# songrise/HyperNeRF-torch

Measured on AMD Instinct MI355X. Metric: ray-samples/sec (fwd+bwd+Adam), whole job; per-GPU = value/n_gpus, higher is better.
Workload: dtype bf16

## Files before the change

### hypernerf-torch_amd/csrc/hn_mlp.hip

```cpp
#include "hn_common.h"
#include <algorithm>
#include <type_traits>

#ifdef HN_PROF
#define HN_STAMP(code)                                                                          \
  do {                                                                                          \
    if (prof_on && prof_n < 2040) {                                                             \
      unsigned long long t__;                                                                   \
      __builtin_amdgcn_sched_barrier(0);                                                        \
      asm volatile("s_memtime %0\n\ts_waitcnt lgkmcnt(0)" : "=s"(t__)::"memory");               \
      __builtin_amdgcn_sched_barrier(0);                                                        \
      if (lane == 0) { prof_buf[2 * prof_n] = (code); prof_buf[2 * prof_n + 1] = (long long)t__; } \
      ++prof_n;                                                                                 \
    }                                                                                           \
  } while (0)
#else
#define HN_STAMP(code) do {} while (0)
#endif

template <int WAVES>
struct WStream {
  const char* g;
  char* lds;
  int ctr;
  int nchunks;
  int wave, lane;

  HN_DEV void issue(int c) {
    const char* src = g + (size_t)c * (HN_CHUNK_UNITS * 1024);
    char* dst = lds + (c & 1) * (HN_CHUNK_UNITS * 1024);
    if constexpr (WAVES == 8) {
      if (wave >= 4) {
        int u0 = wave - 4;
        asm volatile("" : "+s"(u0));
#pragma unroll
        for (int i = 0; i < HN_CHUNK_UNITS / 4; ++i) {
          const int unit = u0 + i * 4;
          __builtin_amdgcn_global_load_lds(
              (const __attribute__((address_space(1))) void*)(src + unit * 1024 + lane * 16),
              (__attribute__((address_space(3))) void*)(dst + unit * 1024), 16, 0, 0);
        }
      }
      return;
    }
#pragma unroll
    for (int i = 0; i < HN_CHUNK_UNITS / WAVES; ++i) {
      const int unit = wave + i * WAVES;
      __builtin_amdgcn_global_load_lds(
          (const __attribute__((address_space(1))) void*)(src + unit * 1024 + lane * 16),
          (__attribute__((address_space(3))) void*)(dst + unit * 1024), 16, 0, 0);
    }
  }
  HN_DEV void start() {
    ctr = 0;
    __syncthreads();
    issue(0);
  }
  HN_DEV const char* take(int n) {
    if ((ctr & (HN_CHUNK_UNITS - 1)) + n > HN_CHUNK_UNITS) ctr = (ctr + HN_CHUNK_UNITS - 1) & ~(HN_CHUNK_UNITS - 1);
    if ((ctr & (HN_CHUNK_UNITS - 1)) == 0) {
      const int c = ctr / HN_CHUNK_UNITS;
      asm volatile("s_waitcnt vmcnt(0)" ::: "memory");
      __syncthreads();
      if (c + 1 < nchunks) issue(c + 1);
    }
    const char* p = lds + (((ctr / HN_CHUNK_UNITS) & 1) * HN_CHUNK_UNITS + (ctr & (HN_CHUNK_UNITS - 1))) * 1024;
    ctr += n;
    return p;
  }
};

#define HN_INV2PI_HI 0.15915494309189535f
#define HN_INV2PI_LO ((float)(0.15915494309189535 - (double)0.15915494309189535f))
HN_DEV void hn_rev_split(float x, float& hi, float& lo) {
  hi = __fmul_rn(x, HN_INV2PI_HI);
  lo = __builtin_fmaf(x, HN_INV2PI_LO, __builtin_fmaf(x, HN_INV2PI_HI, -hi));
}
HN_DEV void hn_stage_sources(float* srcv, const HnMlpArgs& a, int p, int ray, int lane, float* rev = nullptr,
                             int n_trig = 0, bool with_lo = true) {
  const int r = lane & 31, h = lane >> 5;
  for (int ci = h; ci < a.n_comps; ci += 2) {
    const int c = a.comps[ci];
    const int sid = c >> 16, col = c & 0xffff;
    HnSrc s = a.src[0];
    if (sid == 1) s = a.src[1];
    if (sid == 2) s = a.src[2];
    if (sid == 3) s = a.src[3];
    float x = 0.0f;
    if (s.ptr != nullptr) {
      long long row = s.per_ray ? ray : p;
      bool ok = true;
      if (s.gather_idx != nullptr) {
        row = s.gather_idx[ray];
        ok = row >= 0 && row < s.gather_rows;
      }
      x = ok ? s.ptr[(size_t)row * s.ld + col] : __builtin_nanf("");
    }
    srcv[ci * 32 + r] = x;
    if (rev != nullptr && ci < n_trig) {
      float hi, lo;
      hn_rev_split(x, hi, lo);
      rev[ci * 32 + r] = hi;
      if (with_lo) rev[(n_trig + ci) * 32 + r] = lo;
    }
  }
  if (rev != nullptr && !with_lo && h == 0) rev[n_trig * 32 + r] = 0.0f;
}

HN_DEV float hn_direct_source(const HnFeat e, const HnMlpArgs& a, int p, int ray) {
  const int sid = (e.packed >> 8) & 15, col = (e.packed >> 24) & 255;
  const float* base = a.src[0].ptr;
  int ld = a.src[0].ld, pr = a.src[0].per_ray;
  if (sid == 1) { base = a.src[1].ptr; ld = a.src[1].ld; pr = a.src[1].per_ray; }
  if (sid == 2) { base = a.src[2].ptr; ld = a.src[2].ld; pr = a.src[2].per_ray; }
  if (sid == 3) { base = a.src[3].ptr; ld = a.src[3].ld; pr = a.src[3].per_ray; }
  return base[(size_t)(pr ? ray : p) * ld + col];
}

HN_DEV float hn_sin_rev(float t) { return __builtin_amdgcn_sinf(__builtin_amdgcn_fractf(t)); }
#define HN_INV_2PI 0.15915494309189535f

struct HnDFeat { unsigned off; float scale, phase; unsigned idmask; };
HN_DEV HnDFeat hn_derive_feat(const HnFeat e) {
  const int kind = (e.packed >> 12) & 15;
  HnDFeat d;
  d.off = (unsigned)(e.packed & 255) * 128u;
  const bool trig = kind == HN_FEAT_SIN || kind == HN_FEAT_COS || kind == HN_FEAT_SINP;
  d.scale = trig ? e.freq * 0.15915494309189535f : 0.0f;
  d.phase = (kind == HN_FEAT_COS || kind == HN_FEAT_SINP) ? 0.25f : 0.0f;
  d.idmask = (kind == HN_FEAT_ID || kind == HN_FEAT_ID_DIRECT) ? 0xffffffffu : 0u;
  return d;
}
HN_DEV HnDFeat hn_derive_feat_fwd(const HnFeat e, int n_comps, int n_trig, bool with_lo) {
  const int kind = (e.packed >> 12) & 15, ci = e.packed & 255;
  HnDFeat d;
  const bool trig = (kind == HN_FEAT_SIN || kind == HN_FEAT_COS || kind == HN_FEAT_SINP) && ci < n_trig;
  const unsigned oa = trig ? (unsigned)(n_comps + ci) * 128u : (unsigned)ci * 128u;
  const unsigned ob = trig ? (unsigned)(n_comps + n_trig + (with_lo ? ci : 0)) * 128u : oa;
  d.off = oa | ob << 16;
  d.scale = trig ? e.freq : 0.0f;
  d.phase = (kind == HN_FEAT_COS || kind == HN_FEAT_SINP) ? 0.25f : 0.0f;
  d.idmask = (kind == HN_FEAT_ID || kind == HN_FEAT_ID_DIRECT) ? 0xffffffffu : 0u;
  return d;
}
HN_DEV float hn_bfi(unsigned m, float a, float b) {
  return __uint_as_float((m & __float_as_uint(a)) | (~m & __float_as_uint(b)));
}
HN_DEV void hn_features4(const HnDFeat* tp, const char* srcv_r, float* out) {
  u32x4 t[4];
#pragma unroll
  for (int j = 0; j < 4; ++j) t[j] = reinterpret_cast<const u32x4*>(tp)[j];
  __builtin_amdgcn_sched_barrier(0);
  float va[4], vb[4];
// ... 33 lines not shown
  const int kind = (e.packed >> 12) & 15;
  if constexpr (DIRECT) {
    if (kind == HN_FEAT_ID_DIRECT) return hn_direct_source(e, a, p, ray);
  }
  const float x = srcv[(e.packed & 255) * 32 + r];
  if constexpr (BF16) {
    const float ph = (kind == HN_FEAT_COS || kind == HN_FEAT_SINP) ? 0.25f : 0.0f;
    const float s = hn_sin_rev(__builtin_fmaf(e.freq * HN_INV_2PI, x, ph));
    return kind == HN_FEAT_ID ? x : (kind == HN_FEAT_ZERO ? 0.0f : s);
  } else {
    if (kind == HN_FEAT_ZERO) return 0.0f;
    if (kind == HN_FEAT_ID) return x;
    float arg = __fmul_rn(e.freq, x);
    if (kind == HN_FEAT_SINP) arg = __fadd_rn(arg, 0.5f * 3.1415926f);
    return kind == HN_FEAT_COS ? cosf(arg) : sinf(arg);
  }
}

template <bool BF16>
HN_DEV float hn_feature_grad(const HnFeat e, const float* srcv, int r) {
  const int kind = (e.packed >> 12) & 15;
  const float x = srcv[(e.packed & 255) * 32 + r];
  if constexpr (BF16) {
    const float ph = (kind == HN_FEAT_COS || kind == HN_FEAT_SINP) ? 0.5f : 0.25f;
    const float g = e.freq * hn_sin_rev(__builtin_fmaf(e.freq * HN_INV_2PI, x, ph));
    return (kind == HN_FEAT_ID || kind == HN_FEAT_ID_DIRECT) ? 1.0f : g;
  } else {
    if (kind == HN_FEAT_ID || kind == HN_FEAT_ID_DIRECT) return 1.0f;
    float arg = __fmul_rn(e.freq, x);
    if (kind == HN_FEAT_SINP) arg = __fadd_rn(arg, 0.5f * 3.1415926f);
    if (kind == HN_FEAT_COS) return -e.freq * sinf(arg);
    return e.freq * cosf(arg);
  }
}

template <bool DIRECT>
HN_DEV void hn_make_group(bf16x8* out, const HnFeat* ft, const HnDFeat* dft, const float* srcv, int lane,
                          const HnMlpArgs& a, int p, int ray) {
  const int h = lane >> 5, r = lane & 31;
  if constexpr (DIRECT) {
#pragma unroll
    for (int s = 0; s < 4; ++s) {
#pragma unroll
      for (int j = 0; j < 8; ++j)
        out[s][j] = (__bf16)hn_feature<true, true>(ft[16 * s + hn_pi16(h, j)], srcv, r, a, p, ray);
    }
  } else {
    const char* srcv_r = reinterpret_cast<const char*>(srcv) + 4 * r;
#pragma unroll
    for (int s = 0; s < 4; ++s) {
      float v[8];
      hn_features4(dft + 16 * s + 4 * h, srcv_r, v);
      hn_features4(dft + 16 * s + 8 + 4 * h, srcv_r, v + 4);
#pragma unroll
      for (int j = 0; j < 8; ++j) out[s][j] = (__bf16)v[j];
    }
  }
}
template <bool DIRECT>
HN_DEV void hn_make_group(float* out, const HnFeat* ft, const HnDFeat*, const float* srcv, int lane, const HnMlpArgs& a,
                          int p, int ray) {
  const int h = lane >> 5, r = lane & 31;
#pragma unroll
  for (int s = 0; s < 32; ++s) {
    out[s] = hn_feature<false, DIRECT>(ft[32 * (s >> 4) + hn_rho(s & 15, h)], srcv, r, a, p, ray);
    if ((s & 7) == 7) __builtin_amdgcn_sched_barrier(0);
  }
}

HN_DEV void hn_init_acc(f32x16& acc, const float* bias, int t, int h) {
  if (bias != nullptr) {
#pragma unroll
    for (int g = 0; g < 4; ++g) {
      const f32x4 b = *reinterpret_cast<const f32x4*>(bias + 32 * t + 8 * g + 4 * h);
      acc[4 * g] = b[0]; acc[4 * g + 1] = b[1]; acc[4 * g + 2] = b[2]; acc[4 * g + 3] = b[3];
    }
  } else {
#pragma unroll
    for (int i = 0; i < 16; ++i) acc[i] = 0.0f;
  }
}

constexpr int HN_PF = 3;
template <bool BF16, int K32>
HN_DEV void hn_gemm_blocks(f32x16& acc, const typename ModeT<BF16>::Frag* in, WStream<ModeT<BF16>::WAVES>& ws) {
  using M = ModeT<BF16>;
  const char* w = ws.take(K32 * M::UNITS32);
  if constexpr (BF16) {
    constexpr int N = 2 * K32;
    constexpr int D = N < HN_PF ? N : HN_PF;
    const char* wl = w + ws.lane * 16;
    bf16x8 q[D];
#pragma unroll
    for (int u = 0; u < D; ++u) q[u] = *reinterpret_cast<const bf16x8*>(wl + u * 1024);
#pragma unroll
    for (int u = 0; u < N; ++u) {
      acc = hn_mfma_bf16(q[u % D], in[u], acc);
      if (u + D < N) q[u % D] = *reinterpret_cast<const bf16x8*>(wl + (u + D) * 1024);
    }
    __builtin_amdgcn_sched_group_barrier(0x100, D, 0);
#pragma unroll
    for (int u = 0; u < N; ++u) {
      __builtin_amdgcn_sched_group_barrier(0x008, 1, 0);
      if (u + D < N) __builtin_amdgcn_sched_group_barrier(0x100, 1, 0);
    }
  } else {
#pragma unroll
    for (int k = 0; k < K32; ++k) hn_mma_block32(acc, w + k * M::UNITS32 * 1024, in + k * M::STEPS32, ws.lane);
  }
}
template <bool BF16>
HN_DEV void hn_gemm_k(f32x16& acc, const typename ModeT<BF16>::Frag* in, int K32, WStream<ModeT<BF16>::WAVES>& ws) {
  if (K32 == 8) hn_gemm_blocks<BF16, 8>(acc, in, ws);
  else if (K32 == 4) hn_gemm_blocks<BF16, 4>(acc, in, ws);
  else if (K32 == 2) hn_gemm_blocks<BF16, 2>(acc, in, ws);
  else if (K32 == 1) hn_gemm_blocks<BF16, 1>(acc, in, ws);
}

template <bool BF16, int S8 = 0>
HN_DEV char* hn_slot_base(const HnMlpArgs& a, int off_kib, int nt, int blk) {
  if (off_kib < 0) return nullptr;
  constexpr int TU = S8 ? 1 : ModeT<BF16>::TILE_UNITS;
  return reinterpret_cast<char*>(a.stash) + (size_t)(unsigned)off_kib * 1024 + (size_t)blk * nt * (TU * 1024);
}
HN_DEV uint32_t* hn_mask_base(const HnMlpArgs& a, int off256, int nt, int blk, int lane) {
  (void)lane;
  return a.masks + (size_t)(unsigned)off256 * 64 + (size_t)blk * nt * 64;
}
HN_DEV int hn_stash_slot(int r, int h, int u) { return 32 * h + (r ^ (4 * h + 8 * u)); }
HN_DEV int hn_stash8_slot(int r, int h) { return (r & 3) + 4 * h + 8 * ((r >> 2) & 1) + 16 * (r >> 3); }
template <int S8>
HN_DEV int hn_cvt2_f8(unsigned w, int old, bool hi) {
  const float lo_f = __uint_as_float(w << 16), hi_f = __uint_as_float(w & 0xffff0000u);
  if constexpr (S8 == 1) return hi ? __builtin_amdgcn_cvt_pk_fp8_f32(lo_f, hi_f, old, true)
                                   : __builtin_amdgcn_cvt_pk_fp8_f32(lo_f, hi_f, old, false);
  else return hi ? __builtin_amdgcn_cvt_pk_bf8_f32(lo_f, hi_f, old, true)
                 : __builtin_amdgcn_cvt_pk_bf8_f32(lo_f, hi_f, old, false);
}
template <int S8>
HN_DEV void hn_stash8_acc(const f32x16& a, char* slot_base, int t, int lane) {
  u32x4 o;
#pragma unroll
  for (int k = 0; k < 4; ++k) {
    int w = 0;
    if constexpr (S8 == 1) {
      w = __builtin_amdgcn_cvt_pk_fp8_f32(a[4 * k], a[4 * k + 1], w, false);
      w = __builtin_amdgcn_cvt_pk_fp8_f32(a[4 * k + 2], a[4 * k + 3], w, true);
    } else {
      w = __builtin_amdgcn_cvt_pk_bf8_f32(a[4 * k], a[4 * k + 1], w, false);
      w = __builtin_amdgcn_cvt_pk_bf8_f32(a[4 * k + 2], a[4 * k + 3], w, true);
    }
    o[k] = (unsigned)w;
  }
  char* dst8 = slot_base + (size_t)t * 1024 + hn_stash8_slot(lane & 31, lane >> 5) * 16;
  __builtin_nontemporal_store(o, reinterpret_cast<u32x4*>(dst8));
}
template <bool BF16, int S8 = 0>
HN_DEV void hn_stash(const typename ModeT<BF16>::Frag* fr, char* slot_base, int t, int lane) {
  using M = ModeT<BF16>;
  if constexpr (BF16 && S8 != 0) {
    const u32x4 f0 = *reinterpret_cast<const u32x4*>(&fr[0]), f1 = *reinterpret_cast<const u32x4*>(&fr[1]);
    u32x4 o;
#pragma unroll
    for (int k = 0; k < 2; ++k) {
      int lo = 0, hi = 0;
      lo = hn_cvt2_f8<S8>(f0[2 * k], lo, false);
      lo = hn_cvt2_f8<S8>(f0[2 * k + 1], lo, true);
      hi = hn_cvt2_f8<S8>(f1[2 * k], hi, false);
      hi = hn_cvt2_f8<S8>(f1[2 * k + 1], hi, true);
      o[k] = (unsigned)lo;
      o[2 + k] = (unsigned)hi;
    }
    char* dst8 = slot_base + (size_t)t * 1024 + hn_stash8_slot(lane & 31, lane >> 5) * 16;
    __builtin_nontemporal_store(o, reinterpret_cast<u32x4*>(dst8));
    return;
  }
  char* dst = slot_base + (size_t)t * (M::TILE_UNITS * 1024);
  if constexpr (BF16) {
    const int off0 = hn_stash_slot(lane & 31, lane >> 5, 0) * 16;
    __builtin_nontemporal_store(*reinterpret_cast<const u32x4*>(&fr[0]), reinterpret_cast<u32x4*>(dst + off0));
    __builtin_nontemporal_store(*reinterpret_cast<const u32x4*>(&fr[1]), reinterpret_cast<u32x4*>(dst + 1024 + (off0 ^ 128)));
  } else {
    const f32x16 z = hn_transpose_tile(fr, lane);
    hn_store_tile(z, dst, lane, (typename M::Frag*)nullptr);
  }
}

template <bool BF16>
HN_DEV unsigned hn_push_mask(unsigned bits, float x) {
  if constexpr (BF16) return __builtin_amdgcn_alignbit(bits, __float_as_uint(x), 31);
  return (bits << 1) | (x > 0.0f ? 0u : 1u);
}
HN_DEV int hn_keep_mask(unsigned nbits, int q, int i) { return (int)(nbits << (16 * q + i)) >> 31; }

template <bool BF16>
// ... 13 lines not shown
    }
  } else if (act == HN_ACT_SOFTPLUS) {
    const float inv = 1.0f / p0;
#pragma unroll 1
    for (int i = 0; i < 16; ++i) {
      const float z = acc[i], u = z * p0;
      const float sp = BF16 ? __logf(1.0f + __expf(u)) : log1pf(expf(u));
      acc[i] = u > p1 ? z : (BF16 ? sp * inv : sp / p0);
    }
  }
}
template <bool BF16>
HN_DEV float hn_dact_y(int act, float y, float p0, float p1) {
  if (act == HN_ACT_ELU) return y > 0.0f ? 1.0f : y + p0;
  const float u = p0 * y;
  return u > p1 ? 1.0f : (BF16 ? 1.0f - __expf(-u) : -expm1f(-u));
}
template <bool BF16>
HN_DEV f32x16 hn_unstash(const char* slot_base, int t, int lane) {
  using M = ModeT<BF16>;
  const char* src = slot_base + (size_t)t * (M::TILE_UNITS * 1024);
  f32x16 y;
  if constexpr (BF16) {
    const int off0 = hn_stash_slot(lane & 31, lane >> 5, 0) * 16;
    const u32x4 f0 = *reinterpret_cast<const u32x4*>(src + off0);
    const u32x4 f1 = *reinterpret_cast<const u32x4*>(src + 1024 + (off0 ^ 128));
#pragma unroll
    for (int k = 0; k < 4; ++k) {
      y[2 * k] = __uint_as_float(f0[k] << 16);
      y[2 * k + 1] = __uint_as_float(f0[k] & 0xffff0000u);
      y[8 + 2 * k] = __uint_as_float(f1[k] << 16);
      y[8 + 2 * k + 1] = __uint_as_float(f1[k] & 0xffff0000u);
    }
  } else {
    float z[16];
#pragma unroll
    for (int g = 0; g < 4; ++g) {
      const f32x4 v = *reinterpret_cast<const f32x4*>(src + g * 1024 + lane * 16);
#pragma unroll
      for (int e = 0; e < 4; ++e) z[4 * g + e] = v[e];
    }
    y = hn_transpose_tile(z, lane);
  }
  return y;
}

typedef const __attribute__((address_space(4))) int* HnOpPtr;
HN_DEV HnOpPtr hn_op_words(const int* ops, int op) {
  return (HnOpPtr)(uintptr_t)(ops + (size_t)op * HN_OP_WORDS);
}
struct HnOpWords {
  int v[HN_OP_WORDS];
  HN_DEV int operator[](int i) const { return v[i]; }
};
HN_DEV HnOpWords hn_load_op(const int* ops, int op, int n_ops) {
  HnOpWords w;
  const HnOpPtr p = hn_op_words(ops, op < n_ops ? op : n_ops - 1);
#pragma unroll
  for (int i = 0; i < HN_OP_WORDS; ++i) w.v[i] = p[i];
  if (op >= n_ops) w.v[0] = -1;
  return w;
}


template <bool TRAIN, int NT, int S8>
HN_DEV void hn_epilogue_share(int k, int tp, f32x16& a, bf16x8* frag, unsigned& bits, char* out_base,
                              uint32_t* mask_base, int lane) {
  if (k < 8) {
#pragma unroll
    for (int e = 0; e < 2; ++e) {
      const int i = 2 * k + e;
      if (TRAIN) bits = hn_push_mask<true>(bits, a[i]);
      frag[i >> 3][i & 7] = (__bf16)__int_as_float(max(__float_as_int(a[i]), 0));
    }
  } else if (TRAIN && k == 8) {
    hn_stash<true, S8>(frag, out_base, tp, lane);
    if ((tp & 1) || tp == NT - 1) {
      mask_base[(tp >> 1) * 64 + lane] = (tp & 1) ? bits : bits << 16;
      bits = 0;
    }
  }
}

template <int K32, int NT, bool TRAIN, int S8>
HN_DEV void hn_layer_pipelined(bf16x8* cur, bf16x8* nxt, const float* bias, WStream<ModeT<true>::WAVES>& ws,
                               char* out_base, uint32_t* mask_base, int lane) {
  constexpr int N = 2 * K32;
  constexpr int D = 2;
  constexpr int SHARES = 9;
  constexpr int PER_SLOT = (SHARES + N - 1) / N;
  const int h = lane >> 5;
  f32x16 acc[2];
  unsigned bits = 0;
#pragma unroll
  for (int t = 0; t <= NT; ++t) {
    const char* wl = nullptr;
    if (t < NT) wl = ws.take(N) + lane * 16;
    const int tp = t - 1;
    bf16x8 q[D];
    if (t < NT) {
      hn_init_acc(acc[t & 1], bias, t, h);
#pragma unroll
      for (int u = 0; u < D; ++u) q[u] = *reinterpret_cast<const bf16x8*>(wl + u * 1024);
    }
    __builtin_amdgcn_sched_barrier(0);
#pragma unroll
    for (int u = 0; u < N; ++u) {
      if (t < NT) {
        acc[t & 1] = hn_mfma_bf16(q[u % D], cur[u], acc[t & 1]);
        if (u + D < N) q[u % D] = *reinterpret_cast<const bf16x8*>(wl + (u + D) * 1024);
      }
      if (t > 0) {
#pragma unroll
        for (int e = 0; e < PER_SLOT; ++e) {
          const int k = u * PER_SLOT + e;
          if (k < SHARES)
            hn_epilogue_share<TRAIN, NT, S8>(k, tp, acc[tp & 1], nxt + tp * 2, bits, out_base, mask_base, lane);
        }
      }
      __builtin_amdgcn_sched_barrier(0);
    }
  }
#pragma unroll
  for (int i = 0; i < NT * 2; ++i) cur[i] = nxt[i];
}

template <bool BF16, int AUXG, bool EXTRA, bool TRAIN, bool S8 = false>
__global__ __launch_bounds__(ModeT<BF16>::WAVES * 64, BF16 ? 2 : 1) void hn_mlp_fwd_kernel(const HnMlpArgs a) {
  using M = ModeT<BF16>;
  constexpr int SX = S8 ? 1 : 0;
  static_assert(!(S8 && (EXTRA || !TRAIN || !BF16)), "the 8-bit stash exists for the render-level bf16 training builds only");
  if constexpr (S8) asm volatile("s_setreg_imm32_b32 hwreg(HW_REG_MODE, 23, 1), 1");
  using Frag = typename M::Frag;
  extern __shared__ __attribute__((aligned(16))) char smem[];
  const int lane = threadIdx.x & 63;
  const int wave = __builtin_amdgcn_readfirstlane(threadIdx.x >> 6);
  const int r = lane & 31, h = lane >> 5;
  constexpr int PTS = M::WAVES * 32;
  const int ntiles = (a.n_points + PTS - 1) / PTS;
  hn_timeline_begin(a.timeline);
#ifdef HN_PROF
  long long* prof_buf = reinterpret_cast<long long*>(a.prof);
  const bool prof_on = prof_buf != nullptr && blockIdx.x == 0 && wave == 0;
  int prof_n = 0;
#endif

  WStream<M::WAVES> ws;
  ws.g = reinterpret_cast<const char*>(a.wstream);
  ws.lds = smem;
  ws.nchunks = a.n_chunks;
  ws.wave = wave;
  ws.lane = lane;

  Frag cur[8 * M::STEPS32];
  Frag nxt[8 * M::STEPS32];

  float* bias_lds = reinterpret_cast<float*>(smem + 2 * HN_CHUNK_UNITS * 1024);
  HnFeat* feat_lds = reinterpret_cast<HnFeat*>(bias_lds + ((a.n_bias + 3) & ~3));
  HnDFeat* dfeat_lds = reinterpret_cast<HnDFeat*>(feat_lds + ((a.n_feat + 1) & ~1));
  const int n_trig = BF16 ? a.n_trig_comps : 0;
  const bool with_lo = a.trig_lo_planes != 0;
  const int n_planes = BF16 ? a.n_comps + n_trig + (with_lo ? n_trig : 1) : a.n_comps;
  float* srcv = reinterpret_cast<float*>(BF16 ? reinterpret_cast<char*>(dfeat_lds + a.n_feat)
                                              : reinterpret_cast<char*>(dfeat_lds)) + wave * (n_planes * 32);
  float* rev = BF16 ? srcv + a.n_comps * 32 : nullptr;
  for (int i = threadIdx.x; i < a.n_bias; i += blockDim.x) bias_lds[i] = a.bias[i];
  for (int i = threadIdx.x; i < a.n_feat; i += blockDim.x) {
    const HnFeat e = a.feat[i];
    feat_lds[i] = e;
    if constexpr (BF16) dfeat_lds[i] = hn_derive_feat_fwd(e, a.n_comps, n_trig, with_lo);
  }
  __syncthreads();

  for (int tile = blockIdx.x; tile < ntiles; tile += gridDim.x) {
    const int blk = tile * M::WAVES + wave;
    const int p0 = blk * 32 + r;
    const bool valid = p0 < a.n_points;
    const int p = valid ? p0 : a.n_points - 1;
    const int ray = p / a.samples_per_ray;
    const bool wave_valid = blk * 32 < a.n_points;
    hn_stage_sources(srcv, a, p, ray, lane, rev, n_trig, with_lo);
    ws.start();

    HnOpWords w_next = hn_load_op(a.ops, 0, a.n_ops);
    for (int op = 0; op < a.n_ops; ++op) {
      const HnOpWords w = w_next;
      w_next = hn_load_op(a.ops, op + 1, a.n_ops);
      const int code = w[0];
      if (code == HN_OP_LAYER) {
        HN_STAMP(100 + op);
        const int K32 = w[1] & 255, nG = (w[1] >> 8) & 255, NT = (w[1] >> 16) & 255;
        const int act = (w[1] >> 24) & 15, flags = (w[1] >> 28) & 15;
        const float* bias = bias_lds + w[2];
        const bool do_mask = TRAIN && w[4] >= 0 && wave_valid && act != HN_ACT_SOFTPLUS;
        const bool do_stash = TRAIN && w[5] >= 0 && wave_valid;
        char* out_base = do_stash ? hn_slot_base<BF16, SX>(a, w[5], NT, blk) : nullptr;
        char* aux_base = (TRAIN && wave_valid) ? hn_slot_base<BF16, SX>(a, w[6], 2 * nG, blk) : nullptr;
        uint32_t* mask_base = do_mask ? hn_mask_base(a, w[4], (NT + 1) >> 1, blk, lane) : nullptr;
        const bool has_out = w_next[0] == HN_OP_OUT;
        const HnOpWords out_w = w_next;
        Frag aux[AUXG * 2 * M::STEPS32];
#pragma unroll
        for (int g = 0; g < AUXG; ++g) {
          if (g < nG) {
            if (EXTRA && (flags & HN_LAYER_DIRECT))
              hn_make_group<true>(aux + g * 2 * M::STEPS32, feat_lds + w[3] + 64 * g, dfeat_lds + w[3] + 64 * g, srcv,
                                  lane, a, p, ray);
            else
              hn_make_group<false>(aux + g * 2 * M::STEPS32, feat_lds + w[3] + 64 * g, dfeat_lds + w[3] + 64 * g, srcv,
                                   lane, a, p, ray);
            if (aux_base != nullptr) {
              hn_stash<BF16, SX>(aux + g * 2 * M::STEPS32, aux_base, 2 * g, lane);
              hn_stash<BF16, SX>(aux + (g * 2 + 1) * M::STEPS32, aux_base, 2 * g + 1, lane);
            }
          }
        }
        unsigned bits = 0;
        HN_STAMP(1);
        if constexpr (BF16) {
          const bool plain = nG == 0 && act == HN_ACT_RELU && !(flags & HN_LAYER_NO_COMMIT) && !has_out &&
                             wave_valid && do_stash == do_mask;
          if (plain && K32 == 4 && NT == 4) {
            if (do_stash) hn_layer_pipelined<4, 4, true, SX>(cur, nxt, bias, ws, out_base, mask_base, lane);
            else hn_layer_pipelined<4, 4, false, SX>(cur, nxt, bias, ws, out_base, mask_base, lane);
            continue;
          }
        }
#pragma unroll
        for (int t = 0; t < 8; ++t) {
          if (t < NT) {
            f32x16 acc;
            hn_init_acc(acc, bias, t, h);
            hn_gemm_k<BF16>(acc, cur, K32, ws);
#pragma unroll
            for (int g = 0; g < AUXG; ++g)
              if (g < nG) hn_gemm_blocks<BF16, 2>(acc, aux + g * 2 * M::STEPS32, ws);
            HN_STAMP(2);
            if (act == HN_ACT_RELU) {
#pragma unroll
              for (int i = 0; i < 16; ++i) {
                bits = hn_push_mask<BF16>(bits, acc[i]);
                acc[i] = __int_as_float(max(__float_as_int(acc[i]), 0));
              }
            } else if (act != HN_ACT_NONE) {
              hn_act_tile<BF16>(acc, act, __int_as_float(w[7]), __int_as_float(w[4]), bits);
            }
            if (has_out && t == 0 && h == 0 && valid) {
              const HnDst d = a.dst[out_w[1]];
              const int n = out_w[3];
#pragma unroll
              for (int i = 0; i < 4; ++i) {
                if (i < n) {
                  float y = acc[i];
                  if (out_w[4] == 1) y = 1.0f / (1.0f + expf(-y));
                  if (out_w[5] >= 0) {
                    const HnSrc sr = a.src[out_w[5]];
                    y = __fadd_rn(sr.ptr[(size_t)(sr.per_ray ? ray : p) * sr.ld + out_w[6] + i], y);
                  }
                  d.ptr[(size_t)p * d.ld + out_w[2] + i] = y;
                }
              }
            }
            if (has_out && t == 0 && h == 0 && out_w[7] > 0) {
              const int n = out_w[3];
#pragma unroll
              for (int i = 0; i < 4; ++i) {
                if (i < n) {
                  float y = acc[i];
                  if (out_w[4] == 1) y = 1.0f / (1.0f + expf(-y));
                  if (out_w[5] >= 0) {
                    const HnSrc sr = a.src[out_w[5]];
                    y = __fadd_rn(sr.ptr[(size_t)(sr.per_ray ? ray : p) * sr.ld + out_w[6] + i], y);
                  }
                  const int ci = out_w[7] - 1 + i;
                  srcv[ci * 32 + r] = y;
                  if (BF16 && ci < n_trig) {
                    float hi, lo;
                    hn_rev_split(y, hi, lo);
                    rev[ci * 32 + r] = hi;
                    if (with_lo) rev[(n_trig + ci) * 32 + r] = lo;
                  }
                }
              }
            }
            hn_acc_to_frags(acc, nxt + t * M::STEPS32);
#ifdef HN_PROF
            if (prof_on) {
              float x__ = acc[15];
              asm volatile("v_mov_b32 %0, %0" : "+v"(x__)::"memory");
            }
#endif
            HN_STAMP(3);
            if ((t & 1) || t == NT - 1) {
              if (do_mask) mask_base[(t >> 1) * 64 + lane] = (t & 1) ? bits : bits << 16;
              bits = 0;
            }
            if (do_stash) {
              if constexpr (SX != 0) hn_stash8_acc<SX>(acc, out_base, t, lane);
              else hn_stash<BF16, SX>(nxt + t * M::STEPS32, out_base, t, lane);
            }
            HN_STAMP(4);
          }
        }
        if (!(flags & HN_LAYER_NO_COMMIT)) {
#pragma unroll
          for (int t = 0; t < 8; ++t)
            if (t < NT)
#pragma unroll
              for (int s = 0; s < M::STEPS32; ++s) cur[t * M::STEPS32 + s] = nxt[t * M::STEPS32 + s];
        }
      } else if (code == HN_OP_OUT) {
      } else if (EXTRA && code == HN_OP_OUT_WIDE) {
        const int n = w[3], NT = w[4];
        if (valid) {
          const HnDst d = a.dst[w[1]];
#pragma unroll
          for (int t = 0; t < 8; ++t)
            if (t < NT) {
              if constexpr (BF16) {
#pragma unroll
                for (int s = 0; s < 2; ++s)
#pragma unroll
                  for (int j = 0; j < 8; ++j) {
                    const int row = 32 * t + 16 * s + hn_pi16(h, j);
                    if (row < n) d.ptr[(size_t)p * d.ld + w[2] + row] = (float)cur[2 * t + s][j];
                  }
              } else {
#pragma unroll
                for (int q = 0; q < 16; ++q) {
                  const int row = 32 * t + hn_rho(q, h);
                  if (row < n) d.ptr[(size_t)p * d.ld + w[2] + row] = cur[16 * t + q];
                }
              }
            }
        }
      }
    }
  }
  hn_timeline_end(a.timeline);
}

HN_DEV bool hn_prefetch_masks(const HnMlpArgs& a, const HnOpWords& wn, int blk, int lane, bool wave_valid,
                              unsigned* out) {
  if (wn[0] != HN_BOP_LAYER || wn[4] < 0) return false;
  const int NT = (wn[1] >> 16) & 255;
  const uint32_t* mb = hn_mask_base(a, wn[4], (NT + 1) >> 1, blk, lane);
#pragma unroll
  for (int dd = 0; dd < 4; ++dd)
    out[dd] = (2 * dd < NT) ? (wave_valid ? mb[dd * 64 + lane] : 0xffffffffu) : 0u;
  return true;
}

template <bool BF16, bool WIDE, bool S8 = false>
__global__ __launch_bounds__(ModeT<BF16>::WAVES * 64, BF16 ? 2 : 1) void hn_mlp_bwd_kernel(const HnMlpArgs a) {
  using M = ModeT<BF16>;
  constexpr int SZ = S8 ? 2 : 0;
  static_assert(!(S8 && WIDE) && !(S8 && !BF16), "the 8-bit stash exists for the render-level bf16 builds only");
  if constexpr (S8) asm volatile("s_setreg_imm32_b32 hwreg(HW_REG_MODE, 23, 1), 1");
  const float dz_scale = S8 ? ldexpf(1.0f, a.dz_scale_log2) : 1.0f;
  const float dz_unscale = S8 ? ldexpf(1.0f, -a.dz_scale_log2) : 1.0f;
  using Frag = typename M::Frag;
  extern __shared__ __attribute__((aligned(16))) char smem[];
  const int lane = threadIdx.x & 63;
  const int wave = __builtin_amdgcn_readfirstlane(threadIdx.x >> 6);
  const int r = lane & 31, h = lane >> 5;
  constexpr int PTS = M::WAVES * 32;
  const int ntiles = (a.n_points + PTS - 1) / PTS;
  HnFeat* feat_lds = reinterpret_cast<HnFeat*>(smem + 2 * HN_CHUNK_UNITS * 1024);
  HnDFeat* dfeat_lds = reinterpret_cast<HnDFeat*>(feat_lds + ((a.n_feat + 1) & ~1));
  float* srcv = reinterpret_cast<float*>(BF16 ? reinterpret_cast<char*>(dfeat_lds + a.n_feat)
                                              : reinterpret_cast<char*>(dfeat_lds)) + wave * (a.n_comps * 32);
  hn_timeline_begin(a.timeline);
#ifdef HN_PROF
  long long* prof_buf = reinterpret_cast<long long*>(a.prof);
  const bool prof_on = prof_buf != nullptr && blockIdx.x == 0 && wave == 0;
  int prof_n = 0;
#endif
  for (int i = threadIdx.x; i < a.n_feat; i += blockDim.x) {
    const HnFeat e = a.feat[i];
    feat_lds[i] = e;
    if constexpr (BF16) dfeat_lds[i] = hn_derive_feat(e);
  }
  __syncthreads();

  WStream<M::WAVES> ws;
  ws.g = reinterpret_cast<const char*>(a.wstream);
  ws.lds = smem;
  ws.nchunks = a.n_chunks;
  ws.wave = wave;
  ws.lane = lane;

  Frag cur[8 * M::STEPS32];
  Frag nxt[8 * M::STEPS32];
  Frag cur2[M::STEPS32];

  for (int tile = blockIdx.x; tile < ntiles; tile += gridDim.x) {
    const int blk = tile * M::WAVES + wave;
    const int p0 = blk * 32 + r;
    const bool valid = p0 < a.n_points;
    const int p = valid ? p0 : a.n_points - 1;
    const int ray = p / a.samples_per_ray;
    const bool wave_valid = blk * 32 < a.n_points;
    f32x16 dacc;
    hn_init_acc(dacc, nullptr, 0, h);
    hn_stage_sources(srcv, a, p, ray, lane);
    ws.start();

    HnOpWords w_next = hn_load_op(a.ops, 0, a.n_ops);
    unsigned mnext[4] = {0u, 0u, 0u, 0u};
    bool mnext_ready = false;
    for (int op = 0; op < a.n_ops; ++op) {
      const HnOpWords w = w_next;
      w_next = hn_load_op(a.ops, op + 1, a.n_ops);
      const int code = w[0];
      HN_STAMP(100 * code + op);
      if (code != HN_BOP_LAYER && code != HN_BOP_AUX) mnext_ready = false;
      if (code == HN_BOP_LOAD) {
        const int n = w[3] & 255;
        const bool to2 = (w[3] >> 8) & 1;
        float d[4] = {0.f, 0.f, 0.f, 0.f};
        if ((w[3] >> 9) & 1) {
          const int q = (w[3] >> 10) & 3;
#pragma unroll
          for (int i = 0; i < 4; ++i)
            d[i] = q == 0 ? dacc[i] : (q == 1 ? dacc[4 + i] : (q == 2 ? dacc[8 + i] : dacc[12 + i]));
        }
        if (h == 0 && valid) {
          const HnSrc s = a.src[w[1] < 0 ? 0 : w[1]];
#pragma unroll
          for (int i = 0; i < 4; ++i)
            if (i < n) {
              float g = (w[1] >= 0 && s.ptr != nullptr) ? s.ptr[(size_t)p * s.ld + w[2] + i] : 0.0f;
              if constexpr (S8) g *= dz_scale;
              if ((w[3] >> 9) & 1) g += d[i];
              if (w[4] == 1) {
                const HnSrc ys = a.src[w[5]];
                const float y = ys.ptr[(size_t)p * ys.ld + w[6] + i];
                g = g * y * (1.0f - y);
              }
              d[i] = g;
            } else {
              d[i] = 0.0f;
            }
        } else {
#pragma unroll
          for (int i = 0; i < 4; ++i) d[i] = 0.0f;
        }
        Frag tmp[M::STEPS32];
        hn_zero_frags(tmp, M::STEPS32);
        if constexpr (BF16) {
#pragma unroll
          for (int i = 0; i < 4; ++i) tmp[0][i] = (__bf16)d[i];
        } else {
#pragma unroll
          for (int i = 0; i < 4; ++i) tmp[i] = d[i];
        }
        if (a.training && w[7] >= 0 && wave_valid) hn_stash<BF16, SZ>(tmp, hn_slot_base<BF16, SZ>(a, w[7], 1, blk), 0, lane);
#pragma unroll
        for (int s = 0; s < M::STEPS32; ++s) {
          if (to2) cur2[s] = tmp[s];
          else cur[s] = tmp[s];
        }
      } else if (WIDE && code == HN_BOP_LOAD_WIDE) {
        const int n = w[3] & 0xffff, NT = w[4], dact = (w[3] >> 16) & 15;
        const HnSrc s = a.src[w[1]];
        unsigned nbits = 0xffffffffu;
        char* dz_base = (a.training && wave_valid) ? hn_slot_base<BF16>(a, w[7], NT, blk) : nullptr;
        const bool has_mask = w[5] >= 0 && dact != HN_ACT_SOFTPLUS;
        const bool from_y = (dact == HN_ACT_ELU || dact == HN_ACT_SOFTPLUS) && wave_valid;
        const char* y_base = from_y ? hn_slot_base<BF16>(a, w[7], NT, blk) : nullptr;
#pragma unroll
        for (int t = 0; t < 8; ++t) {
          if (t < NT) {
            if (has_mask && !(t & 1)) {
              nbits = wave_valid ? ~hn_mask_base(a, w[5], (NT + 1) >> 1, blk, lane)[(t >> 1) * 64 + lane] : 0u;
            }
            f32x16 v;
            if (dact == 0) {
#pragma unroll
              for (int i = 0; i < 16; ++i) {
                const int row = 32 * t + hn_rho(i, h);
                const bool keep = hn_keep_mask(nbits, t & 1, i) != 0;
                v[i] = (valid && keep && row < n) ? s.ptr[(size_t)p * s.ld + w[2] + row] : 0.0f;
              }
            } else {
              const float p0 = __int_as_float(w[6]), p1 = __int_as_float(w[5]);
              f32x16 y = {0};
              if (y_base != nullptr) y = hn_unstash<BF16>(y_base, t, lane);
#pragma unroll
              for (int i = 0; i < 16; ++i) {
                const int row = 32 * t + hn_rho(i, h);
                const float g = (valid && row < n) ? s.ptr[(size_t)p * s.ld + w[2] + row] : 0.0f;
                float d = 1.0f;
                if (dact == HN_ACT_LEAKY_RELU) d = hn_keep_mask(nbits, t & 1, i) != 0 ? 1.0f : p0;
                else d = hn_dact_y<BF16>(dact, y[i], p0, p1);
                v[i] = g * d;
              }
            }
            hn_acc_to_frags(v, cur + t * M::STEPS32);
            if (dz_base != nullptr) hn_stash<BF16>(cur + t * M::STEPS32, dz_base, t, lane);
          }
        }
      } else if (code == HN_BOP_LAYER) {
        const int K32 = w[1] & 255, K32b = (w[1] >> 8) & 255, NT = (w[1] >> 16) & 255;
        const bool has_mask = w[4] >= 0;
        const bool do_stash = a.training && w[5] >= 0 && wave_valid;
        char* dz_base = do_stash ? hn_slot_base<BF16, SZ>(a, w[5], NT, blk) : nullptr;
        const int dact = w[2];
        const char* y_base = (!S8 && (dact == HN_ACT_ELU || dact == HN_ACT_SOFTPLUS) && wave_valid)
                                 ? hn_slot_base<BF16>(a, w[6], NT, blk) : nullptr;
        unsigned nbits = 0xffffffffu;
        unsigned mbits[4] = {0xffffffffu, 0xffffffffu, 0xffffffffu, 0xffffffffu};
        if (has_mask) {
          if (mnext_ready) {
#pragma unroll
            for (int dd = 0; dd < 4; ++dd) mbits[dd] = ~mnext[dd];
          } else {
            const uint32_t* mb = hn_mask_base(a, w[4], (NT + 1) >> 1, blk, lane);
#pragma unroll
            for (int dd = 0; dd < 4; ++dd)
              if (2 * dd < NT)
                mbits[dd] = wave_valid ? ~mb[dd * 64 + lane] : 0u;
          }
        }
        mnext_ready = false;
#pragma unroll
        for (int t = 0; t < 8; ++t) {
          if (t < NT) {
            f32x16 acc;
            hn_init_acc(acc, nullptr, t, h);
            hn_gemm_k<BF16>(acc, cur, K32, ws);
            if (K32b) hn_gemm_blocks<BF16, 1>(acc, cur2, ws);
            if (t == 0) mnext_ready = hn_prefetch_masks(a, w_next, blk, lane, wave_valid, mnext);
            HN_STAMP(2);
            if (!(t & 1)) nbits = mbits[t >> 1];
            if (dact == 0) {
#pragma unroll
              for (int i = 0; i < 16; ++i)
                acc[i] = __int_as_float(__float_as_int(acc[i]) & hn_keep_mask(nbits, t & 1, i));
            } else if (dact == HN_ACT_LEAKY_RELU) {
              const float p0 = __int_as_float(w[3]);
#pragma unroll
              for (int i = 0; i < 16; ++i)
                if (hn_keep_mask(nbits, t & 1, i) == 0) acc[i] *= p0;
            } else if (y_base != nullptr) {
              const f32x16 y = hn_unstash<BF16>(y_base, t, lane);
              const float p0 = __int_as_float(w[3]), p1 = __int_as_float(w[7]);
#pragma unroll
              for (int i = 0; i < 16; ++i) acc[i] *= hn_dact_y<BF16>(dact, y[i], p0, p1);
            }
            hn_acc_to_frags(acc, nxt + t * M::STEPS32);
            if (do_stash) {
              if constexpr (SZ != 0) hn_stash8_acc<SZ>(acc, dz_base, t, lane);
              else hn_stash<BF16, SZ>(nxt + t * M::STEPS32, dz_base, t, lane);
            }
            HN_STAMP(4);
          }
        }
#pragma unroll
        for (int t = 0; t < 8; ++t)
          if (t < NT)
#pragma unroll
            for (int s = 0; s < M::STEPS32; ++s) cur[t * M::STEPS32 + s] = nxt[t * M::STEPS32 + s];
      } else if (code == HN_BOP_AUX) {
        const int K32 = w[1] & 255, K32b = (w[1] >> 8) & 255, nG = (w[1] >> 16) & 255;
        const int tiles = w[2];
        bool first = true;
        mnext_ready = false;
        for (int tt = 0; tt < 2 * nG; ++tt) {
          if (!((tiles >> tt) & 1)) continue;
          f32x16 acc;
          hn_init_acc(acc, nullptr, 0, h);
          hn_gemm_k<BF16>(acc, cur, K32, ws);
          if (K32b) hn_gemm_blocks<BF16, 1>(acc, cur2, ws);
          if (first) mnext_ready = hn_prefetch_masks(a, w_next, blk, lane, wave_valid, mnext);
          first = false;
          const HnFeat* ft = feat_lds + w[3] + 32 * tt;
          if ((tiles >> (8 + tt)) & 1) {
            if constexpr (BF16) {
              const HnDFeat* dft = dfeat_lds + w[3] + 32 * tt + 4 * h;
              const char* srcv_r = reinterpret_cast<const char*>(srcv) + 4 * r;
#pragma unroll
              for (int q4 = 0; q4 < 4; ++q4) {
                float g[4];
                hn_feature_grads4(dft + 8 * q4, srcv_r, g);
#pragma unroll
                for (int e = 0; e < 4; ++e) acc[4 * q4 + e] *= g[e];
              }
            } else {
#pragma unroll
              for (int i = 0; i < 16; ++i) acc[i] *= hn_feature_grad<BF16>(ft[hn_rho(i, h)], srcv, r);
            }
          }
          Frag gfr[M::STEPS32];
          hn_acc_to_frags(acc, gfr);
          hn_gemm_blocks<BF16, 1>(dacc, gfr, ws);
          HN_STAMP(5);
        }
      }
    }
    if (a.n_dsrc > 0 && a.dsrc != nullptr && p0 < a.n_points) {
#pragma unroll
      for (int i = 0; i < 16; ++i) {
        const int slot = hn_rho(i, h);
        if (slot < a.n_dsrc) a.dsrc[(size_t)p0 * a.n_dsrc + slot] = S8 ? dacc[i] * dz_unscale : dacc[i];
      }
    }
    if (a.embed_reg_mask != 0 && wave_valid) {
      const long long erow = a.embed_idx[(blk * 32) / a.samples_per_ray];
#pragma unroll
      for (int i = 0; i < 16; ++i) {
        if (a.embed_reg_mask & (1 << i)) {
          float v = valid ? (S8 ? dacc[i] * dz_unscale : dacc[i]) : 0.0f;
#pragma unroll
          for (int m = 1; m < 32; m <<= 1) v += __shfl_xor(v, m, 64);
          const int col = a.embed_col[hn_rho(i, h)];
          if (r == 0 && col >= 0) {
            if (!S8 && a.embed_partial != nullptr) a.embed_partial[(size_t)blk * a.embed_dim + col] = v;
            else if (erow >= 0 && erow < a.embed_rows) atomicAdd(a.embed_grad + (size_t)erow * a.embed_dim + col, v);
          }
        }
      }
    }
  }
  hn_timeline_end(a.timeline);
}

#include "hn_pack.h"
template <bool BF16>
__global__ void hn_pack_kernel(const HnPackUnit* units, int n_units, const float* const* ptrs, char* out,
                               const HnPackBias* bias, int n_bias, float* bias_out) {
  hn_pack_one<BF16>(units, n_units, ptrs, out, bias, n_bias, bias_out, blockIdx.x * (blockDim.x >> 6) + (threadIdx.x >> 6));
}
template <bool BF16>
__global__ void hn_pack_multi_kernel(const HnPackTable tab) {
  hn_pack_block<BF16>(tab, (int)blockIdx.x);
}

template <class F>
HN_DEV void static_for4(F&& f) {
  f(std::integral_constant<int, 0>{});
  f(std::integral_constant<int, 1>{});
  f(std::integral_constant<int, 2>{});
  f(std::integral_constant<int, 3>{});
}
template <bool BF16>
struct DwFrag;
typedef __attribute__((ext_vector_type(4))) short s16x4;
typedef __attribute__((ext_vector_type(8))) short s16x8;
HN_DEV void hn_dw_tr_offsets(int lane, int& o0, int& o1) {
  const int G = lane >> 4, i = lane & 15, q = i >> 2, pp = i & 3;
  const int u = G & 1, hh = G >> 1, h = pp & 1, g = pp >> 1;
  o0 = u * 1024 + hn_stash_slot(8 * hh + q, h, u) * 16 + 8 * g;
  o1 = u * 1024 + hn_stash_slot(8 * hh + 4 + q, h, u) * 16 + 8 * g;
}
typedef __attribute__((ext_vector_type(2))) unsigned int u32x2;
template <int NZ>
HN_DEV void hn_tr_block(bf16x8 (*x)[2], bf16x8 (*z)[2], unsigned ax0, unsigned ax1, unsigned az0, unsigned az1) {
  u32x2 r[8 + 4 * NZ];
  if constexpr (NZ == 4) {
    asm volatile(
        "ds_read_b64_tr_b16 %0, %24\n\t"
        "ds_read_b64_tr_b16 %1, %25\n\t"
        "ds_read_b64_tr_b16 %2, %24 offset:256\n\t"
        "ds_read_b64_tr_b16 %3, %25 offset:256\n\t"
        "ds_read_b64_tr_b16 %4, %24 offset:2048\n\t"
        "ds_read_b64_tr_b16 %5, %25 offset:2048\n\t"
        "ds_read_b64_tr_b16 %6, %24 offset:2304\n\t"
        "ds_read_b64_tr_b16 %7, %25 offset:2304\n\t"
        "ds_read_b64_tr_b16 %8, %26\n\t"
        "ds_read_b64_tr_b16 %9, %27\n\t"
        "ds_read_b64_tr_b16 %10, %26 offset:256\n\t"
        "ds_read_b64_tr_b16 %11, %27 offset:256\n\t"
        "ds_read_b64_tr_b16 %12, %26 offset:2048\n\t"
        "ds_read_b64_tr_b16 %13, %27 offset:2048\n\t"
        "ds_read_b64_tr_b16 %14, %26 offset:2304\n\t"
        "ds_read_b64_tr_b16 %15, %27 offset:2304\n\t"
        "ds_read_b64_tr_b16 %16, %26 offset:4096\n\t"
        "ds_read_b64_tr_b16 %17, %27 offset:4096\n\t"
        "ds_read_b64_tr_b16 %18, %26 offset:4352\n\t"
        "ds_read_b64_tr_b16 %19, %27 offset:4352\n\t"
// ... 1046 lines not shown
```

Baseline: 82.62 million.

## Defer weight-stream DMA waits until global stores and use lighter barriers

For bf16 kernels, the weight-stream chunk rendezvous no longer forces s_waitcnt vmcnt(0) on every wave. Only the waves that issued the global-to-LDS DMA track a pending flag and wait, and an explicit confirm() drains it before any global store (stash, mask, output), since vmcnt also counts stores. The __syncthreads is replaced by an lgkmcnt wait plus a raw s_barrier. Optional profiling instrumentation (HN_PROF_RDV) is also added. This cuts stalls at chunk boundaries but risks ordering hazards if some store or LDS read path lacks a confirm.

```diff
diff --git a/hypernerf-torch_amd/csrc/hn_mlp.hip b/hypernerf-torch_amd/csrc/hn_mlp.hip
--- a/hypernerf-torch_amd/csrc/hn_mlp.hip
+++ b/hypernerf-torch_amd/csrc/hn_mlp.hip
@@ -17,14 +17,24 @@
 #else
 #define HN_STAMP(code) do {} while (0)
 #endif
-
-template <int WAVES>
+#ifdef HN_PROF_RDV
+#undef HN_STAMP
+#define HN_STAMP(code) do {} while (0)
+#define HN_RDV_TS(x) asm volatile("s_memtime %0\n\ts_waitcnt lgkmcnt(0)" : "=s"(x)::"memory")
+#endif
+
+template <int WAVES, bool KEEP>
 struct WStream {
   const char* g;
   char* lds;
   int ctr;
   int nchunks;
   int wave, lane;
+  int dma_pending;
+#ifdef HN_PROF_RDV
+  unsigned long long rdv_wait = 0, rdv_bar = 0, rdv_dma = 0;
+  int rdv_n = 0;
+#endif
 
   HN_DEV void issue(int c) {
     const char* src = g + (size_t)c * (HN_CHUNK_UNITS * 1024);
@@ -51,24 +61,85 @@
           (__attribute__((address_space(3))) void*)(dst + unit * 1024), 16, 0, 0);
     }
   }
+  HN_DEV bool issuer() const { return WAVES != 8 || wave >= 4; }
+  HN_DEV void barrier() {
+    if constexpr (!KEEP) {
+      __syncthreads();
+      return;
+    }
+    asm volatile("s_waitcnt lgkmcnt(0)" ::: "memory");
+    __builtin_amdgcn_s_barrier();
+    __builtin_amdgcn_sched_barrier(0);
+    asm volatile("" ::: "memory");
+  }
+  HN_DEV void confirm() {
+    if constexpr (!KEEP) return;
+    if (dma_pending) {
+#ifdef HN_PROF_RDV
+      unsigned long long t0_, t1_;
+      HN_RDV_TS(t0_);
+#endif
+      asm volatile("s_waitcnt vmcnt(0)" ::: "memory");
+#ifdef HN_PROF_RDV
+      HN_RDV_TS(t1_);
+      rdv_dma += t1_ - t0_;
+#endif
+      dma_pending = 0;
+    }
+  }
   HN_DEV void start() {
     ctr = 0;
-    __syncthreads();
+    barrier();
     issue(0);
+    if constexpr (KEEP) dma_pending = issuer();
   }
   HN_DEV const char* take(int n) {
     if ((ctr & (HN_CHUNK_UNITS - 1)) + n > HN_CHUNK_UNITS) ctr = (ctr + HN_CHUNK_UNITS - 1) & ~(HN_CHUNK_UNITS - 1);
     if ((ctr & (HN_CHUNK_UNITS - 1)) == 0) {
       const int c = ctr / HN_CHUNK_UNITS;
-      asm volatile("s_waitcnt vmcnt(0)" ::: "memory");
-      __syncthreads();
-      if (c + 1 < nchunks) issue(c + 1);
+#ifdef HN_PROF_RDV
+      unsigned long long t0_, t1_, t2_;
+      HN_RDV_TS(t0_);
+#endif
+      if constexpr (!KEEP) {
+        asm volatile("s_waitcnt vmcnt(0)" ::: "memory");
+      } else if (dma_pending) {
+        asm volatile("s_waitcnt vmcnt(0)" ::: "memory");
+        dma_pending = 0;
+      }
+#ifdef HN_PROF_RDV
+      HN_RDV_TS(t1_);
+#endif
+      barrier();
+#ifdef HN_PROF_RDV
+      HN_RDV_TS(t2_);
+      rdv_wait += t1_ - t0_; rdv_bar += t2_ - t1_; ++rdv_n;
+#endif
+      if (c + 1 < nchunks) {
+        issue(c + 1);
+        if constexpr (KEEP) dma_pending = issuer();
+      }
     }
     const char* p = lds + (((ctr / HN_CHUNK_UNITS) & 1) * HN_CHUNK_UNITS + (ctr & (HN_CHUNK_UNITS - 1))) * 1024;
     ctr += n;
     return p;
   }
 };
+
+#ifdef HN_PROF_RDV
+template <class WS>
+HN_DEV void hn_rdv_record(long long* buf, int& n, long long code, unsigned long long t_start, WS& ws) {
+  unsigned long long t_end;
+  HN_RDV_TS(t_end);
+  if (n < 255 && ws.lane == 0) {
+    long long* q = buf + (ws.wave == 0 ? 0 : 2048) + 8 * n;
+    q[0] = code; q[1] = (long long)ws.rdv_wait; q[2] = (long long)ws.rdv_bar; q[3] = (long long)ws.rdv_dma;
+    q[4] = (long long)(t_end - t_start); q[5] = ws.rdv_n;
+  }
+  ++n;
+  ws.rdv_wait = ws.rdv_bar = ws.rdv_dma = 0; ws.rdv_n = 0;
+}
+#endif
 
 #define HN_INV2PI_HI 0.15915494309189535f
 #define HN_INV2PI_LO ((float)(0.15915494309189535 - (double)0.15915494309189535f))
@@ -268,8 +339,8 @@
 }
 
 constexpr int HN_PF = 3;
-template <bool BF16, int K32>
-HN_DEV void hn_gemm_blocks(f32x16& acc, const typename ModeT<BF16>::Frag* in, WStream<ModeT<BF16>::WAVES>& ws) {
+template <bool BF16, int K32, class WS>
+HN_DEV void hn_gemm_blocks(f32x16& acc, const typename ModeT<BF16>::Frag* in, WS& ws) {
   using M = ModeT<BF16>;
   const char* w = ws.take(K32 * M::UNITS32);
   if constexpr (BF16) {
@@ -295,8 +366,8 @@
     for (int k = 0; k < K32; ++k) hn_mma_block32(acc, w + k * M::UNITS32 * 1024, in + k * M::STEPS32, ws.lane);
   }
 }
-template <bool BF16>
-HN_DEV void hn_gemm_k(f32x16& acc, const typename ModeT<BF16>::Frag* in, int K32, WStream<ModeT<BF16>::WAVES>& ws) {
+template <bool BF16, class WS>
+HN_DEV void hn_gemm_k(f32x16& acc, const typename ModeT<BF16>::Frag* in, int K32, WS& ws) {
   if (K32 == 8) hn_gemm_blocks<BF16, 8>(acc, in, ws);
   else if (K32 == 4) hn_gemm_blocks<BF16, 4>(acc, in, ws);
   else if (K32 == 2) hn_gemm_blocks<BF16, 2>(acc, in, ws);
@@ -476,8 +547,8 @@
   }
 }
 
-template <int K32, int NT, bool TRAIN, int S8>
-HN_DEV void hn_layer_pipelined(bf16x8* cur, bf16x8* nxt, const float* bias, WStream<ModeT<true>::WAVES>& ws,
+template <int K32, int NT, bool TRAIN, int S8, class WS>
+HN_DEV void hn_layer_pipelined(bf16x8* cur, bf16x8* nxt, const float* bias, WS& ws,
                                char* out_base, uint32_t* mask_base, int lane) {
   constexpr int N = 2 * K32;
   constexpr int D = 2;
@@ -505,6 +576,7 @@
         if (u + D < N) q[u % D] = *reinterpret_cast<const bf16x8*>(wl + (u + D) * 1024);
       }
       if (t > 0) {
+        if (TRAIN && u * PER_SLOT <= 8 && 8 < (u + 1) * PER_SLOT) ws.confirm();
 #pragma unroll
         for (int e = 0; e < PER_SLOT; ++e) {
           const int k = u * PER_SLOT + e;
@@ -538,13 +610,19 @@
   const bool prof_on = prof_buf != nullptr && blockIdx.x == 0 && wave == 0;
   int prof_n = 0;
 #endif
-
-  WStream<M::WAVES> ws;
+#ifdef HN_PROF_RDV
+  const bool rdv_on = prof_buf != nullptr && blockIdx.x == 0 && (wave == 0 || wave == 4);
+  int rdv_rec = 0;
+  unsigned long long rdv_t0 = 0;
+#endif
+
+  WStream<M::WAVES, BF16> ws;
   ws.g = reinterpret_cast<const char*>(a.wstream);
   ws.lds = smem;
   ws.nchunks = a.n_chunks;
   ws.wave = wave;
   ws.lane = lane;
+  ws.dma_pending = 0;
 
   Frag cur[8 * M::STEPS32];
   Frag nxt[8 * M::STEPS32];
@@ -584,6 +662,10 @@
       if (code == HN_OP_LAYER) {
         HN_STAMP(100 + op);
         const int K32 = w[1] & 255, nG = (w[1] >> 8) & 255, NT = (w[1] >> 16) & 255;
+#ifdef HN_PROF_RDV
+        if (rdv_on) HN_RDV_TS(rdv_t0);
+        const long long rdv_code = 1ll << 32 | (long long)NT << 24 | nG << 16 | K32 << 8 | op;
+#endif
         const int act = (w[1] >> 24) & 15, flags = (w[1] >> 28) & 15;
         const float* bias = bias_lds + w[2];
         const bool do_mask = TRAIN && w[4] >= 0 && wave_valid && act != HN_ACT_SOFTPLUS;
@@ -604,6 +686,7 @@
               hn_make_group<false>(aux + g * 2 * M::STEPS32, feat_lds + w[3] + 64 * g, dfeat_lds + w[3] + 64 * g, srcv,
                                    lane, a, p, ray);
             if (aux_base != nullptr) {
+              ws.confirm();
               hn_stash<BF16, SX>(aux + g * 2 * M::STEPS32, aux_base, 2 * g, lane);
               hn_stash<BF16, SX>(aux + (g * 2 + 1) * M::STEPS32, aux_base, 2 * g + 1, lane);
             }
@@ -617,6 +700,9 @@
           if (plain && K32 == 4 && NT == 4) {
             if (do_stash) hn_layer_pipelined<4, 4, true, SX>(cur, nxt, bias, ws, out_base, mask_base, lane);
             else hn_layer_pipelined<4, 4, false, SX>(cur, nxt, bias, ws, out_base, mask_base, lane);
+#ifdef HN_PROF_RDV
+            if (rdv_on) hn_rdv_record(prof_buf, rdv_rec, rdv_code | 1ll << 40, rdv_t0, ws);
+#endif
             continue;
           }
         }
@@ -639,6 +725,7 @@
             } else if (act != HN_ACT_NONE) {
               hn_act_tile<BF16>(acc, act, __int_as_float(w[7]), __int_as_float(w[4]), bits);
             }
+            if (TRAIN && has_out && t == 0) ws.confirm();
             if (has_out && t == 0 && h == 0 && valid) {
               const HnDst d = a.dst[out_w[1]];
               const int n = out_w[3];
@@ -685,6 +772,7 @@
             }
 #endif
             HN_STAMP(3);
+            if constexpr (TRAIN) ws.confirm();
             if ((t & 1) || t == NT - 1) {
               if (do_mask) mask_base[(t >> 1) * 64 + lane] = (t & 1) ? bits : bits << 16;
               bits = 0;
@@ -703,6 +791,9 @@
 #pragma unroll
               for (int s = 0; s < M::STEPS32; ++s) cur[t * M::STEPS32 + s] = nxt[t * M::STEPS32 + s];
         }
+#ifdef HN_PROF_RDV
+        if (rdv_on) hn_rdv_record(prof_buf, rdv_rec, rdv_code, rdv_t0, ws);
+#endif
       } else if (code == HN_OP_OUT) {
       } else if (EXTRA && code == HN_OP_OUT_WIDE) {
         const int n = w[3], NT = w[4];
@@ -770,6 +861,11 @@
   const bool prof_on = prof_buf != nullptr && blockIdx.x == 0 && wave == 0;
   int prof_n = 0;
 #endif
+#ifdef HN_PROF_RDV
+  const bool rdv_on = prof_buf != nullptr && blockIdx.x == 0 && (wave == 0 || wave == 4);
+  int rdv_rec = 0;
+  unsigned long long rdv_t0 = 0;
+#endif
   for (int i = threadIdx.x; i < a.n_feat; i += blockDim.x) {
     const HnFeat e = a.feat[i];
     feat_lds[i] = e;
@@ -777,12 +873,13 @@
   }
   __syncthreads();
 
-  WStream<M::WAVES> ws;
+  WStream<M::WAVES, BF16 && !S8> ws;
   ws.g = reinterpret_cast<const char*>(a.wstream);
   ws.lds = smem;
   ws.nchunks = a.n_chunks;
   ws.wave = wave;
   ws.lane = lane;
+  ws.dma_pending = 0;
 
   Frag cur[8 * M::STEPS32];
   Frag nxt[8 * M::STEPS32];
@@ -808,6 +905,9 @@
       w_next = hn_load_op(a.ops, op + 1, a.n_ops);
       const int code = w[0];
       HN_STAMP(100 * code + op);
+#ifdef HN_PROF_RDV
+      if (rdv_on) HN_RDV_TS(rdv_t0);
+#endif
       if (code != HN_BOP_LAYER && code != HN_BOP_AUX) mnext_ready = false;
       if (code == HN_BOP_LOAD) {
         const int n = w[3] & 255;
@@ -849,7 +949,10 @@
 #pragma unroll
           for (int i = 0; i < 4; ++i) tmp[i] = d[i];
         }
-        if (a.training && w[7] >= 0 && wave_valid) hn_stash<BF16, SZ>(tmp, hn_slot_base<BF16, SZ>(a, w[7], 1, blk), 0, lane);
+        if (a.training && w[7] >= 0 && wave_valid) {
+          ws.confirm();
+          hn_stash<BF16, SZ>(tmp, hn_slot_base<BF16, SZ>(a, w[7], 1, blk), 0, lane);
+        }
 #pragma unroll
         for (int s = 0; s < M::STEPS32; ++s) {
           if (to2) cur2[s] = tmp[s];
@@ -945,6 +1048,7 @@
             }
             hn_acc_to_frags(acc, nxt + t * M::STEPS32);
             if (do_stash) {
+              ws.confirm();
               if constexpr (SZ != 0) hn_stash8_acc<SZ>(acc, dz_base, t, lane);
               else hn_stash<BF16, SZ>(nxt + t * M::STEPS32, dz_base, t, lane);
             }
@@ -956,6 +1060,9 @@
           if (t < NT)
 #pragma unroll
             for (int s = 0; s < M::STEPS32; ++s) cur[t * M::STEPS32 + s] = nxt[t * M::STEPS32 + s];
+#ifdef HN_PROF_RDV
+        if (rdv_on) hn_rdv_record(prof_buf, rdv_rec, 2ll << 32 | (long long)NT << 24 | K32b << 16 | K32 << 8 | op, rdv_t0, ws);
+#endif
       } else if (code == HN_BOP_AUX) {
         const int K32 = w[1] & 255, K32b = (w[1] >> 8) & 255, nG = (w[1] >> 16) & 255;
         const int tiles = w[2];
@@ -991,6 +1098,9 @@
           hn_gemm_blocks<BF16, 1>(dacc, gfr, ws);
           HN_STAMP(5);
         }
+#ifdef HN_PROF_RDV
+        if (rdv_on) hn_rdv_record(prof_buf, rdv_rec, 3ll << 32 | (long long)(2 * nG) << 24 | K32b << 16 | K32 << 8 | op, rdv_t0, ws);
+#endif
       }
     }
     if (a.n_dsrc > 0 && a.dsrc != nullptr && p0 < a.n_points) {
```

Result: slower. 81.76 million (-1.1%).
